# showlab/VideoSwap

Measured on AMD Instinct MI355X. Metric: denoised frames/sec, 16-frame 512x512 clip @ 50 DDIM steps (end to end: inversion + CFG sampling), higher is better.
Workload: dtype f16; 1 GPU; BASELINE.json configs[1]: 16-frame 512x512 clip, SD-1.5 UNet3D + AnimateDiff motion modules, 50-step DDIM inversion (B=1) + 50-step CFG-7.5 DDIM sampling (B=2), 1 clip per GPU per step; launch=eager, parallelism=clip-parallel x1

## Files before the change

include/vsx.h:

```cpp
#ifndef VSX_H_
#define VSX_H_

#include <stddef.h>
#include <stdint.h>

#ifdef __cplusplus
extern "C" {
#endif

#define VSX_ABI_VERSION 13

#define VSX_OK 0
#define VSX_E_BADSHAPE (-1)
#define VSX_E_UNSUPPORTED (-2)
#define VSX_E_LAUNCH (-3)
#define VSX_E_WORKSPACE (-4)

typedef void* vsx_stream_t;

int vsx_abi_version(void);
const char* vsx_last_error(void);
const char* vsx_source_digest(void);
int vsx_set_option(const char* name, int64_t value);

typedef struct vsx_gemm_desc {
    int64_t M, N, K;
    int64_t batch0, batch1;

    const void* A;
    const void* A2;
    int64_t lda, a_bs0, a_bs1;
    int64_t a_mode;
    int64_t H, W;
    int64_t C1, C2;
    int64_t ks, stride;
    int64_t upsample;

    const void* B;
    int64_t ldb, b_bs0, b_bs1;

    void* C;
    int64_t ldc, c_bs0, c_bs1;
    int64_t c_mode;
    int64_t c_rows_per_img;
    int64_t c_img_stride;

    const void* bias;
    const void* rowvec;
    int64_t rows_per_vec;
    const void* residual;
    int64_t ldr, r_bs0, r_bs1;
    int64_t geglu;
    double alpha;
    void* workspace;
    int64_t workspace_bytes;
    int64_t pad_lo, pad_hi;
    const void* rowscale;
    const void* colvec;
    void* rowstats;
    int64_t rowstats_parts;
} vsx_gemm_desc;

int vsx_gemm_f16(const vsx_gemm_desc* d, vsx_stream_t stream);
int64_t vsx_gemm_rowstats_parts(const vsx_gemm_desc* d);
int64_t vsx_gemm_workspace(const vsx_gemm_desc* d);

int64_t vsx_groupnorm_chunks(int64_t rows, int64_t nimg);
int vsx_groupnorm_stats(const void* x1, const void* x2, int64_t nimg, int64_t rows, int64_t C1,
                        int64_t C2, int64_t groups, float* partial, vsx_stream_t stream);
int vsx_groupnorm_apply(const void* x1, const void* x2, int64_t nimg, int64_t rows, int64_t C1,
                        int64_t C2, int64_t groups, const float* partial, int64_t nchunks,
                        int64_t count_rows, const void* gamma, const void* beta, float eps,
                        int64_t silu, float* stats, void* y, vsx_stream_t stream);

int vsx_row_stats(const void* x, int64_t M, int64_t C, float eps, float* stats, vsx_stream_t stream);
int vsx_row_stats_combine(const float* parts, int64_t M, int64_t nparts, int64_t C, float eps, float* stats,
                          vsx_stream_t stream);

int vsx_layernorm(const void* x, int64_t M, int64_t C, const void* gamma, const void* beta,
                  float eps, const void* pe, int64_t rows_per_frame, int64_t frames,
                  int64_t frame_offset, void* y, vsx_stream_t stream);

int vsx_attention_f16(const void* Q, const void* K, const void* VT, void* O, int64_t nb,
                      int64_t heads, int64_t nq, int64_t nk, int64_t d, int64_t ldq, int64_t ldk,
                      int64_t ldvt, int64_t ldo, int64_t q_bs, int64_t k_bs, int64_t vt_bs,
                      int64_t o_bs, int64_t kv_div, float scale, vsx_stream_t stream);

int vsx_attention_lse_f16(const void* Q, const void* K, const void* VT, void* O, float* lse, int64_t lse_ld, int64_t nb,
                          int64_t heads, int64_t nq, int64_t nk, int64_t d, int64_t ldq, int64_t ldk, int64_t ldvt,
                          int64_t ldo, int64_t q_bs, int64_t k_bs, int64_t vt_bs, int64_t o_bs, int64_t kv_div,
                          float scale, vsx_stream_t stream);
int64_t vsx_attention_bwd_supported(int64_t d);
int vsx_attention_bwd_f16(const void* Q, const void* K, const void* V, const void* O, const void* dO, const void* QT,
                          const void* KT, const void* dOT, const float* lse, float* delta, void* dQ, void* dK, void* dV,
                          int64_t nb, int64_t heads, int64_t nq, int64_t nk, int64_t d, int64_t ldtq, int64_t ldtk,
                          int64_t lds, int64_t kv_div, float scale, vsx_stream_t stream);

int vsx_softmax_rows(void* S, int64_t nrows, int64_t ncols, int64_t ld, vsx_stream_t stream);
int vsx_softmax_rows_causal(void* S, int64_t nrows, int64_t ncols, int64_t ld, int64_t rows_per_seq,
                            vsx_stream_t stream);

int vsx_temporal_attention_f16(const void* Q, const void* K, const void* V, void* O, int64_t B,
                               int64_t fq, int64_t fk, int64_t hw, int64_t heads, int64_t d,
                               int64_t ldq, int64_t ldkv, int64_t ldo, float scale,
                               vsx_stream_t stream);

int vsx_silu(const void* x, void* y, int64_t n, vsx_stream_t stream);
int vsx_quick_gelu(const void* x, void* y, int64_t n, vsx_stream_t stream);
int vsx_axpy(const void* a, const void* b, float s, void* y, int64_t n, vsx_stream_t stream);
int vsx_pack_latents(const void* x, void* y, int64_t B, int64_t Cin, int64_t F, int64_t HW,
                     int64_t Cpad, vsx_stream_t stream);
int vsx_unpack_latents(const void* x, void* y, int64_t B, int64_t Cout, int64_t F, int64_t HW,
                       int64_t Cs, vsx_stream_t stream);
int vsx_cfg_ddim_step(const void* x, const void* eps_u, const void* eps_c, float guidance,
                      float alpha_t, float alpha_next, void* out, int64_t n, vsx_stream_t stream);
int vsx_masked_blend(const void* x, const void* src, const void* mask, void* out, int64_t C,
                     int64_t n_sp, vsx_stream_t stream);

int vsx_adapter_scatter(const float* tracks, const int32_t* selected, const void* feat, void* out,
                        int64_t F, int64_t P, int64_t C, int64_t h, int64_t w, float rate,
                        float out_scale, vsx_stream_t stream);

int vsx_prof_enable(int64_t on, int64_t max_samples);
int vsx_prof_pause(int64_t paused);
int vsx_prof_collect(int64_t* n_launches, double* total_ms, double* total_flop);
int vsx_prof_collect_roofline(double peak_flops, double peak_bytes_per_s, int64_t* n_launches, double* total_ms,
                              double* total_flop, double* total_bytes, double* floor_ms, double* byte_bound_ms);

#define VSX_COMM_OP_SEND 1
#define VSX_COMM_OP_RECV 2
#define VSX_COMM_OP_ALLGATHER 3
#define VSX_COMM_OP_ALLREDUCE 4
#define VSX_COMM_OP_LOCAL_COPY 5
#define VSX_COMM_OP_GROUP_START 6
#define VSX_COMM_OP_GROUP_END 7
int vsx_comm_unique_id(void* id128);
int vsx_comm_init(int64_t rank, int64_t nranks, const void* id128);
int vsx_comm_init_recording(int64_t rank, int64_t nranks);
int64_t vsx_comm_recorded(int64_t* out, int64_t capacity);
int64_t vsx_comm_size(void);
int64_t vsx_comm_rank(void);
int vsx_comm_destroy(void);
int vsx_allgather_kv(const void* kv_local, void* kv_all, int64_t batch, int64_t elems_per_batch,
                     vsx_stream_t stream);
int vsx_allgather_f32(const float* local, float* all, int64_t count, vsx_stream_t stream);
int vsx_allreduce_gnstats(float* partial, int64_t count, vsx_stream_t stream);
int vsx_alltoall_f16(const void* send, void* recv, int64_t nouter, int64_t ninner, int64_t block_elems,
                     const int64_t* send_strides, const int64_t* recv_strides, vsx_stream_t stream);

int vsx_geglu_fwd(const void* y2, void* out, int64_t M, int64_t N, vsx_stream_t stream);
int vsx_geglu_bwd(const void* dout, const void* y2, void* dy2, int64_t M, int64_t N, vsx_stream_t stream);
int vsx_silu_bwd(const void* dy, const void* x, void* dx, int64_t n, vsx_stream_t stream);
int64_t vsx_groupnorm_bwd_workspace(int64_t nimg, int64_t rows, int64_t groups);
int vsx_groupnorm_bwd(const void* dy, const void* x1, const void* x2, int64_t nimg, int64_t rows, int64_t C1,
                      int64_t C2, int64_t groups, const void* gamma, const void* beta, float eps, int64_t silu,
                      void* ws, void* dx1, void* dx2, vsx_stream_t stream);
// ... 37 lines not shown
```

videoswap_amd/_lib.py:

```python
import ctypes
import os
from ctypes import POINTER, Structure, c_char_p, c_double, c_float, c_int, c_int32, c_int64, c_void_p

_HERE = os.path.dirname(os.path.abspath(__file__))
VARIANT = os.environ.get('VSX_LIB_VARIANT') or None
LIB_PATH = os.path.join(_HERE, 'lib', 'libvsx.so' if not VARIANT else f'libvsx_{VARIANT}.so')

VSX_ABI_VERSION = 13
VSX_E_UNSUPPORTED = -2


class VsxError(RuntimeError):
    pass


class GemmDesc(Structure):

    def __init__(self, *args, **kwargs):
        super().__init__(*args, **kwargs)
        if 'pad_lo' not in kwargs:
            self.pad_lo = -1
        if 'pad_hi' not in kwargs:
            self.pad_hi = -1

    _fields_ = [
        ('M', c_int64), ('N', c_int64), ('K', c_int64),
        ('batch0', c_int64), ('batch1', c_int64),
        ('A', c_void_p), ('A2', c_void_p),
        ('lda', c_int64), ('a_bs0', c_int64), ('a_bs1', c_int64),
        ('a_mode', c_int64), ('H', c_int64), ('W', c_int64), ('C1', c_int64), ('C2', c_int64),
        ('ks', c_int64), ('stride', c_int64), ('upsample', c_int64),
        ('B', c_void_p), ('ldb', c_int64), ('b_bs0', c_int64), ('b_bs1', c_int64),
        ('C', c_void_p), ('ldc', c_int64), ('c_bs0', c_int64), ('c_bs1', c_int64),
        ('c_mode', c_int64), ('c_rows_per_img', c_int64), ('c_img_stride', c_int64),
        ('bias', c_void_p), ('rowvec', c_void_p), ('rows_per_vec', c_int64),
        ('residual', c_void_p), ('ldr', c_int64), ('r_bs0', c_int64), ('r_bs1', c_int64),
        ('geglu', c_int64), ('alpha', c_double),
        ('workspace', c_void_p), ('workspace_bytes', c_int64),
        ('pad_lo', c_int64), ('pad_hi', c_int64),
        ('rowscale', c_void_p), ('colvec', c_void_p),
        ('rowstats', c_void_p), ('rowstats_parts', c_int64),
    ]


PROTOTYPES = {
    'vsx_abi_version': (c_int, []),
    'vsx_last_error': (c_char_p, []),
    'vsx_source_digest': (c_char_p, []),
    'vsx_set_option': (c_int, [c_char_p, c_int64]),
    'vsx_gemm_f16': (c_int, [POINTER(GemmDesc), c_void_p]),
    'vsx_gemm_workspace': (c_int64, [POINTER(GemmDesc)]),
    'vsx_gemm_rowstats_parts': (c_int64, [POINTER(GemmDesc)]),
    'vsx_groupnorm_chunks': (c_int64, [c_int64, c_int64]),
    'vsx_groupnorm_stats': (c_int, [c_void_p, c_void_p, c_int64, c_int64, c_int64, c_int64, c_int64, c_void_p,
                                    c_void_p]),
    'vsx_groupnorm_apply': (c_int, [c_void_p, c_void_p, c_int64, c_int64, c_int64, c_int64, c_int64, c_void_p,
                                    c_int64, c_int64, c_void_p, c_void_p, c_float, c_int64, c_void_p, c_void_p, c_void_p]),
    'vsx_row_stats': (c_int, [c_void_p, c_int64, c_int64, c_float, c_void_p, c_void_p]),
    'vsx_row_stats_combine': (c_int, [c_void_p, c_int64, c_int64, c_int64, c_float, c_void_p, c_void_p]),
    'vsx_layernorm': (c_int, [c_void_p, c_int64, c_int64, c_void_p, c_void_p, c_float, c_void_p, c_int64, c_int64,
                              c_int64, c_void_p, c_void_p]),
    'vsx_attention_f16': (c_int, [c_void_p, c_void_p, c_void_p, c_void_p] + [c_int64] * 14 + [c_float, c_void_p]),
    'vsx_attention_lse_f16': (c_int, [c_void_p, c_void_p, c_void_p, c_void_p, c_void_p] + [c_int64] * 15 + [c_float, c_void_p]),
    'vsx_attention_bwd_supported': (c_int64, [c_int64]),
    'vsx_attention_bwd_f16': (c_int, [c_void_p] * 13 + [c_int64] * 9 + [c_float, c_void_p]),
    'vsx_softmax_rows': (c_int, [c_void_p, c_int64, c_int64, c_int64, c_void_p]),
    'vsx_softmax_rows_causal': (c_int, [c_void_p, c_int64, c_int64, c_int64, c_int64, c_void_p]),
    'vsx_temporal_attention_f16': (c_int, [c_void_p, c_void_p, c_void_p, c_void_p] + [c_int64] * 9
                                   + [c_float, c_void_p]),
    'vsx_silu': (c_int, [c_void_p, c_void_p, c_int64, c_void_p]),
    'vsx_quick_gelu': (c_int, [c_void_p, c_void_p, c_int64, c_void_p]),
    'vsx_axpy': (c_int, [c_void_p, c_void_p, c_float, c_void_p, c_int64, c_void_p]),
    'vsx_pack_latents': (c_int, [c_void_p, c_void_p, c_int64, c_int64, c_int64, c_int64, c_int64, c_void_p]),
    'vsx_unpack_latents': (c_int, [c_void_p, c_void_p, c_int64, c_int64, c_int64, c_int64, c_int64, c_void_p]),
    'vsx_cfg_ddim_step': (c_int, [c_void_p, c_void_p, c_void_p, c_float, c_float, c_float, c_void_p, c_int64,
                                  c_void_p]),
    'vsx_masked_blend': (c_int, [c_void_p, c_void_p, c_void_p, c_void_p, c_int64, c_int64, c_void_p]),
    'vsx_adapter_scatter': (c_int, [c_void_p, c_void_p, c_void_p, c_void_p, c_int64, c_int64, c_int64, c_int64,
                                    c_int64, c_float, c_float, c_void_p]),
    'vsx_prof_enable': (c_int, [c_int64, c_int64]),
    'vsx_comm_unique_id': (c_int, [c_void_p]),
    'vsx_comm_init': (c_int, [c_int64, c_int64, c_void_p]),
    'vsx_comm_init_recording': (c_int, [c_int64, c_int64]),
    'vsx_comm_recorded': (c_int64, [POINTER(c_int64), c_int64]),
    'vsx_comm_size': (c_int64, []),
    'vsx_comm_rank': (c_int64, []),
    'vsx_comm_destroy': (c_int, []),
    'vsx_allgather_kv': (c_int, [c_void_p, c_void_p, c_int64, c_int64, c_void_p]),
    'vsx_allgather_f32': (c_int, [c_void_p, c_void_p, c_int64, c_void_p]),
    'vsx_allreduce_gnstats': (c_int, [c_void_p, c_int64, c_void_p]),
    'vsx_prof_pause': (c_int, [c_int64]),
    'vsx_prof_collect': (c_int, [POINTER(c_int64), POINTER(c_double), POINTER(c_double)]),
    'vsx_prof_collect_roofline': (c_int, [c_double, c_double, POINTER(c_int64), POINTER(c_double), POINTER(c_double),
                                          POINTER(c_double), POINTER(c_double), POINTER(c_double)]),
    'vsx_geglu_fwd': (c_int, [c_void_p, c_void_p, c_int64, c_int64, c_void_p]),
    'vsx_geglu_bwd': (c_int, [c_void_p, c_void_p, c_void_p, c_int64, c_int64, c_void_p]),
    'vsx_silu_bwd': (c_int, [c_void_p, c_void_p, c_void_p, c_int64, c_void_p]),
    'vsx_groupnorm_bwd_workspace': (c_int64, [c_int64, c_int64, c_int64]),
    'vsx_groupnorm_bwd': (c_int, [c_void_p, c_void_p, c_void_p, c_int64, c_int64, c_int64, c_int64, c_int64, c_void_p,
                                  c_void_p, c_float, c_int64, c_void_p, c_void_p, c_void_p, c_void_p]),
    'vsx_layernorm_bwd': (c_int, [c_void_p, c_void_p, c_void_p, c_float, c_void_p, c_int64, c_int64, c_void_p]),
    'vsx_softmax_bwd': (c_int, [c_void_p, c_void_p, c_int64, c_int64, c_int64, c_float, c_void_p]),
    'vsx_sum_pool2x2': (c_int, [c_void_p, c_void_p, c_int64, c_int64, c_int64, c_int64, c_void_p]),
    'vsx_adapter_gather': (c_int, [c_void_p, c_void_p, c_void_p, c_void_p, c_int64, c_int64, c_int64, c_int64, c_int64,
                                   c_float, c_float, c_void_p]),
    'vsx_alltoall_f16': (c_int, [c_void_p, c_void_p, c_int64, c_int64, c_int64, POINTER(c_int64), POINTER(c_int64),
                                 c_void_p]),
    'vsx_dift_sample_points': (c_int, [c_void_p] + [c_int64] * 7 + [c_void_p, c_int64, c_void_p, c_int64, c_void_p,
                                                                       c_void_p, c_void_p]),
    'vsx_dift_cosine_map_workspace': (c_int64, [c_int64] * 5),
    'vsx_dift_cosine_map': (c_int, [c_void_p] + [c_int64] * 7 + [c_void_p, c_int64, c_int64, c_void_p, c_int64,
                                                                    c_void_p, c_void_p, c_void_p, c_void_p]),
    'vsx_coord_mlp_f32': (c_int, [c_void_p] + [c_int64] * 10 + [c_void_p, c_int64, c_void_p, c_void_p]),
    'vsx_hash_grid_geometry': (c_int64, [c_int64] * 4 + [c_double] + [c_void_p] * 5),
    'vsx_hash_grid_f32': (c_int, [c_void_p, c_int64, c_int64, c_void_p] + [c_int64] * 5 + [c_double, c_void_p, c_void_p]),
    'vsx_hash_mlp_f32': (c_int, [c_void_p, c_int64, c_int64, c_void_p] + [c_int64] * 5 + [c_double] + [c_int64] * 5
                         + [c_void_p, c_int64, c_void_p, c_void_p]),
}

OPTIONAL_PROTOTYPES = {}

_lib = None


def load():
    global _lib
    if _lib is not None:
        return _lib
    if not os.path.exists(LIB_PATH):
        raise VsxError(
            f'{LIB_PATH} not found: the HIP extension is the only implementation of the denoising path; '
            f'build it with `python -m videoswap_amd.build` (hipcc --offload-arch=gfx950).')
    lib = ctypes.CDLL(LIB_PATH)
    for name, (restype, argtypes) in PROTOTYPES.items():
        fn = getattr(lib, name)
        fn.restype = restype
        fn.argtypes = argtypes
    for name, (restype, argtypes) in OPTIONAL_PROTOTYPES.items():
        fn = getattr(lib, name, None)
        if fn is not None:
# ... 22 lines not shown
```

videoswap_amd/csrc/norm.hip:

```cpp
#include "common.h"
#include "options.h"

namespace {

constexpr int GN_MAX_THREADS = 512;
constexpr int GN_MAX_GROUPS = 64;

__host__ __device__ inline int gn_threads(int C) {
    const int vpr = C >> 3;
    return (GN_MAX_THREADS / vpr) * vpr;
}

__host__ __device__ inline int gn_stat_rows(long rows, long nimg) {
    long r = rows * nimg / 768;
    return (int)(r < 8 ? 8 : (r > 1024 ? 1024 : r));
}
__host__ __device__ inline int gn_apply_rows(long rows, long nimg) {
    long r = rows * nimg / 1024;
    return (int)(r < 4 ? 4 : (r > 512 ? 512 : r));
}

__device__ __forceinline__ int gn_col(const int c, const int C) { return ((c >> 2) & 1) * (C >> 1) + (c >> 3) * 4 + (c & 3); }

__device__ __forceinline__ const half_t* gn_src(const half_t* x1, const half_t* x2, int c, int C1, int C2, long& pitch) {
// ... 110 lines not shown
                                                                  const float* __restrict__ stats,
                                                                  const half_t* __restrict__ gamma, const half_t* __restrict__ beta,
                                                                  int silu, half_t* __restrict__ y, const float* __restrict__ partial,
                                                                  int nchunks, float inv_count, float eps, float* __restrict__ stats_out) {
    const int C = C1 + C2;
    const int cpg = C / groups;
    const int vpr = C >> 3;
    const int rp = (int)blockDim.x / vpr;
    const int tid = threadIdx.x;
    const int rl = tid / vpr;
    const int c0 = (tid - rl * vpr) * 8;
    const long img = blockIdx.y;
    __shared__ float st_sh[FUSED ? 2 * GN_MAX_GROUPS : 2];
    if constexpr (FUSED) {
        const int lane = tid & 63, wave = tid >> 6;
        const int nwaves = (int)blockDim.x >> 6;
        if (wave < nwaves) {
            const float2* pp = reinterpret_cast<const float2*>(partial) + img * nchunks * groups;
            for (int g = wave; g < groups; g += nwaves) {
                float2 v = lane < nchunks ? pp[(long)lane * groups + g] : make_float2(0.f, 0.f);
#pragma unroll
                for (int w = 32; w > 0; w >>= 1) {
                    v.x += __shfl_down(v.x, w, 64);
                    v.y += __shfl_down(v.y, w, 64);
                }
                if (lane == 0) {
                    float mean, rstd;
                    gn_mean_rstd(v.x, v.y, inv_count, eps, mean, rstd);
                    st_sh[2 * g] = mean;
                    st_sh[2 * g + 1] = rstd;
                    if (blockIdx.x == 0) {
                        stats_out[(img * groups + g) * 2] = mean;
                        stats_out[(img * groups + g) * 2 + 1] = rstd;
                    }
                }
            }
        }
        __syncthreads();
    }
    float ca[8], cb[8];
    {
        const h8 gm = as_h8(ld16(gamma + c0)), bt = as_h8(ld16(beta + c0));
        const float* st = FUSED ? st_sh : stats + img * groups * 2;
        int g = c0 / cpg, left = (g + 1) * cpg - c0;
        float mean = st[2 * g], rstd = st[2 * g + 1];
#pragma unroll
        for (int e = 0; e < 8; ++e) {
            if (left == 0) { ++g; left = cpg; mean = st[2 * g]; rstd = st[2 * g + 1]; }
            --left;
            ca[e] = rstd * (float)gm[e];
            cb[e] = (float)bt[e] - mean * ca[e];
        }
    }
    long pitch;
    const half_t* src = gn_src(x1, x2, c0, C1, C2, pitch) + img * rows * pitch;
    half_t* dst = y + img * rows * C + c0;
    const int rpb = gn_apply_rows(rows, gridDim.y);
    const long r0 = (long)blockIdx.x * rpb;
    const long r1 = min(r0 + (long)rpb, rows);
    for (long rb = r0 + rl; rb < r1; rb += 4 * rp) {
        uint4 raw[4];
#pragma unroll
        for (int u = 0; u < 4; ++u) {
            const long r = rb + u * rp;
            raw[u] = r < r1 ? ld16(src + r * pitch) : make_uint4(0, 0, 0, 0);
        }
#pragma unroll
        for (int u = 0; u < 4; ++u) {
            const long r = rb + u * rp;
            if (r >= r1) break;
            const h8 v = as_h8(raw[u]);
            h8 o;
#pragma unroll
            for (int e = 0; e < 8; ++e) {
                float f = __builtin_fmaf((float)v[e], ca[e], cb[e]);
                if (silu) f = silu_f(f);
                o[e] = (half_t)f;
            }
            st16(dst + r * C, as_u4(o));
        }
    }
}

template <int NV, int R>
__global__ __launch_bounds__(256) void layernorm_kernel(const half_t* __restrict__ x, long M, int C,
                                                        const half_t* __restrict__ gamma,
                                                        const half_t* __restrict__ beta, float eps,
                                                        const half_t* __restrict__ pe, long rows_per_frame, int frames,
                                                        int frame_offset, half_t* __restrict__ y) {
    const int lane = threadIdx.x & 63;
    const long m0 = ((long)blockIdx.x * 4 + (threadIdx.x >> 6)) * R;
    if (m0 >= M) return;
    const int vpr = C >> 3;
    uint4 raw[R][NV];
#pragma unroll
    for (int r = 0; r < R; ++r)
#pragma unroll
        for (int k = 0; k < NV; ++k) {
            const int v = lane + 64 * k;
            raw[r][k] = (v < vpr && m0 + r < M) ? ld16(x + (m0 + r) * C + v * 8) : make_uint4(0, 0, 0, 0);
        }
    h8 gm[NV], bt[NV];
#pragma unroll
    for (int k = 0; k < NV; ++k) {
        const int v = lane + 64 * k;
        if (v < vpr) {
            gm[k] = as_h8(ld16(gamma + v * 8));
            bt[k] = as_h8(ld16(beta + v * 8));
        }
    }
#pragma unroll
    for (int r = 0; r < R; ++r) {
        const long m = m0 + r;
        if (m >= M) break;
        float f[NV][8];
        float sum = 0.f;
#pragma unroll
        for (int k = 0; k < NV; ++k) {
            const h8 h = as_h8(raw[r][k]);
#pragma unroll
            for (int e = 0; e < 8; ++e) { f[k][e] = (float)h[e]; sum += f[k][e]; }
        }
        const float mean = wave_sum(sum) / (float)C;
        float sq = 0.f;
#pragma unroll
        for (int k = 0; k < NV; ++k) {
            if (lane + 64 * k < vpr) {
#pragma unroll
                for (int e = 0; e < 8; ++e) { const float d = f[k][e] - mean; sq += d * d; }
            }
        }
        const float rstd = rsqrtf(wave_sum(sq) / (float)C + eps);
        const half_t* perow = nullptr;
        if (pe) {
            const long fr = (m / rows_per_frame) % frames + frame_offset;
            perow = pe + fr * C;
        }
#pragma unroll
        for (int k = 0; k < NV; ++k) {
            const int v = lane + 64 * k;
            if (v < vpr) {
                h8 o;
                if (perow) {
                    const h8 pv = as_h8(ld16(perow + v * 8));
#pragma unroll
                    for (int e = 0; e < 8; ++e)
                        o[e] = (half_t)((f[k][e] - mean) * rstd * (float)gm[k][e] + (float)bt[k][e] + (float)pv[e]);
                } else {
#pragma unroll
                    for (int e = 0; e < 8; ++e)
                        o[e] = (half_t)((f[k][e] - mean) * rstd * (float)gm[k][e] + (float)bt[k][e]);
                }
                st16(y + m * C + v * 8, as_u4(o));
            }
        }
    }
}

template <int NV, int R>
__global__ __launch_bounds__(256) void row_stats_kernel(const half_t* __restrict__ x, long M, int C, float eps,
                                                        float* __restrict__ stats) {
    const int lane = threadIdx.x & 63;
    const long m0 = ((long)blockIdx.x * 4 + (threadIdx.x >> 6)) * R;
    if (m0 >= M) return;
    const int vpr = C >> 3;
    uint4 raw[R][NV];
// ... 63 lines not shown
    for (int c = lane; c < ncols; c += 64) sum += __expf((float)row[c] - mx);
    sum = wave_sum(sum);
    const float inv = 1.0f / sum;
    for (int c = lane; c < ncols; c += 64) row[c] = (half_t)(__expf((float)row[c] - mx) * inv);
}

__global__ __launch_bounds__(256) void softmax_rows_causal_kernel(half_t* __restrict__ S, long nrows, int ncols,
                                                                  long ld, int rows_per_seq) {
    const int lane = threadIdx.x & 63;
    const long r = (long)blockIdx.x * 4 + (threadIdx.x >> 6);
    if (r >= nrows) return;
    half_t* row = S + r * ld;
    const int live = min(ncols, (int)(r % rows_per_seq) + 1);
    float mx = -INFINITY;
    for (int c = lane; c < live; c += 64) mx = fmaxf(mx, (float)row[c]);
    mx = wave_max(mx);
    float sum = 0.f;
    for (int c = lane; c < live; c += 64) sum += __expf((float)row[c] - mx);
    sum = wave_sum(sum);
    const float inv = 1.0f / sum;
    for (int c = lane; c < ncols; c += 64) row[c] = c < live ? (half_t)(__expf((float)row[c] - mx) * inv) : (half_t)0.f;
}

}

extern "C" int64_t vsx_groupnorm_chunks(int64_t rows, int64_t nimg) {
    const int rpc = gn_stat_rows(rows, nimg);
    return (rows + rpc - 1) / rpc;
}

static int gn_check(const void* x1, const void* x2, int64_t nimg, int64_t rows, int64_t C1, int64_t C2,
                    int64_t groups) {
    VSX_REQUIRE(x1 && nimg > 0 && rows > 0, VSX_E_BADSHAPE, "groupnorm: empty input");
    VSX_REQUIRE(C1 > 0 && C1 % 8 == 0 && C2 >= 0 && C2 % 8 == 0, VSX_E_BADSHAPE,
                "groupnorm: channels must be multiples of 8 (C1=%ld C2=%ld)", (long)C1, (long)C2);
    VSX_REQUIRE((C2 == 0) == (x2 == nullptr), VSX_E_BADSHAPE, "groupnorm: x2/C2 mismatch");
    const int64_t C = C1 + C2;
    VSX_REQUIRE(C <= 4096, VSX_E_UNSUPPORTED, "groupnorm: C=%ld > 4096", (long)C);
    VSX_REQUIRE(groups > 0 && groups <= GN_MAX_GROUPS && C % groups == 0, VSX_E_BADSHAPE,
                "groupnorm: groups=%ld does not divide C=%ld (max %d groups)", (long)groups, (long)C, GN_MAX_GROUPS);
    VSX_REQUIRE(vsx_aligned16(x1) && vsx_aligned16(x2), VSX_E_BADSHAPE, "groupnorm: inputs must be 16-byte aligned");
    VSX_REQUIRE(nimg <= 65535, VSX_E_BADSHAPE, "groupnorm: nimg=%ld > 65535", (long)nimg);
    return VSX_OK;
}

extern "C" int vsx_groupnorm_stats(const void* x1, const void* x2, int64_t nimg, int64_t rows, int64_t C1,
                                   int64_t C2, int64_t groups, float* partial, vsx_stream_t stream) {
    int rc = gn_check(x1, x2, nimg, rows, C1, C2, groups);
    if (rc) return rc;
    VSX_REQUIRE(partial != nullptr, VSX_E_WORKSPACE, "groupnorm_stats: null partial buffer");
    dim3 grid((unsigned)vsx_groupnorm_chunks(rows, nimg), (unsigned)nimg);
    hipLaunchKernelGGL(gn_stats_kernel, grid, dim3((unsigned)gn_threads((int)(C1 + C2))), 0, (hipStream_t)stream, (const half_t*)x1,
                       (const half_t*)x2, (long)rows, (int)C1, (int)C2, (int)groups, partial);
    return vsx_check_launch("vsx_groupnorm_stats");
}

extern "C" int vsx_groupnorm_apply(const void* x1, const void* x2, int64_t nimg, int64_t rows, int64_t C1,
                                   int64_t C2, int64_t groups, const float* partial, int64_t nchunks,
                                   int64_t count_rows, const void* gamma, const void* beta, float eps, int64_t silu,
                                   float* stats, void* y, vsx_stream_t stream) {
    int rc = gn_check(x1, x2, nimg, rows, C1, C2, groups);
    if (rc) return rc;
    VSX_REQUIRE(partial && gamma && beta && y && stats, VSX_E_BADSHAPE, "groupnorm_apply: null argument");
    VSX_REQUIRE(nchunks > 0 && count_rows > 0, VSX_E_BADSHAPE, "groupnorm_apply: nchunks/count_rows");
    VSX_REQUIRE(vsx_aligned16(gamma) && vsx_aligned16(beta) && vsx_aligned16(y), VSX_E_BADSHAPE,
                "groupnorm_apply: gamma/beta/y must be 16-byte aligned");
    const int64_t C = C1 + C2;
    const float inv_count = 1.0f / ((float)count_rows * (float)(C / groups));
    const int rpb = gn_apply_rows(rows, nimg);
    dim3 grid((unsigned)((rows + rpb - 1) / rpb), (unsigned)nimg);
    const unsigned threads = (unsigned)gn_threads((int)C);
    if (nchunks <= GN_FUSE_MAX_CHUNKS && threads >= 64 && vsxg::gemm_option("gn_fuse") != 0) {
        hipLaunchKernelGGL(gn_apply_kernel<true>, grid, dim3(threads), 0, (hipStream_t)stream, (const half_t*)x1, (const half_t*)x2,
                           (long)rows, (int)C1, (int)C2, (int)groups, (const float*)nullptr, (const half_t*)gamma, (const half_t*)beta,
                           (int)silu, (half_t*)y, partial, (int)nchunks, inv_count, eps, stats);
        return vsx_check_launch("vsx_groupnorm_apply");
    }
    hipLaunchKernelGGL(gn_finalize_kernel, dim3((unsigned)groups, (unsigned)nimg), dim3(256), 0, (hipStream_t)stream, partial,
                       (int)nchunks, (int)groups, inv_count, eps, stats);
    hipLaunchKernelGGL(gn_apply_kernel<false>, grid, dim3(threads), 0, (hipStream_t)stream, (const half_t*)x1, (const half_t*)x2,
                       (long)rows, (int)C1, (int)C2, (int)groups, stats, (const half_t*)gamma, (const half_t*)beta,
                       (int)silu, (half_t*)y, (const float*)nullptr, 0, 0.f, 0.f, (float*)nullptr);
    return vsx_check_launch("vsx_groupnorm_apply");
}

extern "C" int vsx_layernorm(const void* x, int64_t M, int64_t C, const void* gamma, const void* beta, float eps,
                             const void* pe, int64_t rows_per_frame, int64_t frames, int64_t frame_offset, void* y,
                             vsx_stream_t stream) {
    VSX_REQUIRE(x && gamma && beta && y, VSX_E_BADSHAPE, "layernorm: null argument");
    if (M == 0) return VSX_OK;
    VSX_REQUIRE(M > 0 && C > 0 && C % 8 == 0 && C <= 2048, VSX_E_BADSHAPE, "layernorm: C=%ld must be a multiple of 8, <= 2048",
                (long)C);
    VSX_REQUIRE(vsx_aligned16(x) && vsx_aligned16(gamma) && vsx_aligned16(beta) && vsx_aligned16(y) && vsx_aligned16(pe),
                VSX_E_BADSHAPE, "layernorm: pointers must be 16-byte aligned");
    if (pe) VSX_REQUIRE(rows_per_frame > 0 && frames > 0 && frame_offset >= 0, VSX_E_BADSHAPE, "layernorm: pe geometry");
    const long rpf = rows_per_frame > 0 ? rows_per_frame : 1;
    const int nfr = (int)(frames > 0 ? frames : 1);
#define VSX_LN_LAUNCH(NV, R)                                                                                            \
    hipLaunchKernelGGL((layernorm_kernel<NV, R>), dim3((unsigned)((M + 4 * (R) - 1) / (4 * (R)))), dim3(256), 0,            \
                       (hipStream_t)stream, (const half_t*)x, (long)M, (int)C, (const half_t*)gamma,                    \
                       (const half_t*)beta, eps, (const half_t*)pe, rpf, nfr, (int)frame_offset, (half_t*)y)
    if (C <= 512) VSX_LN_LAUNCH(1, 4);
    else if (C <= 1024) VSX_LN_LAUNCH(2, 2);
    else VSX_LN_LAUNCH(4, 1);
#undef VSX_LN_LAUNCH
    return vsx_check_launch("vsx_layernorm");
}

extern "C" int vsx_row_stats(const void* x, int64_t M, int64_t C, float eps, float* stats, vsx_stream_t stream) {
    VSX_REQUIRE(x && stats, VSX_E_BADSHAPE, "row_stats: null argument");
    if (M == 0) return VSX_OK;
    VSX_REQUIRE(M > 0 && C > 0 && C % 8 == 0 && C <= 2048, VSX_E_BADSHAPE, "row_stats: C=%ld must be a multiple of 8, <= 2048",
                (long)C);
    VSX_REQUIRE(vsx_aligned16(x), VSX_E_BADSHAPE, "row_stats: x must be 16-byte aligned");
#define VSX_RS_LAUNCH(NV, R)                                                                                            \
    hipLaunchKernelGGL((row_stats_kernel<NV, R>), dim3((unsigned)((M + 4 * (R) - 1) / (4 * (R)))), dim3(256), 0,            \
                       (hipStream_t)stream, (const half_t*)x, (long)M, (int)C, eps, stats)
    if (C <= 512) VSX_RS_LAUNCH(1, 4);
    else if (C <= 1024) VSX_RS_LAUNCH(2, 2);
    else VSX_RS_LAUNCH(4, 1);
#undef VSX_RS_LAUNCH
    return vsx_check_launch("vsx_row_stats");
}

extern "C" int vsx_row_stats_combine(const float* parts, int64_t M, int64_t nparts, int64_t C, float eps, float* stats,
                                     vsx_stream_t stream) {
    VSX_REQUIRE(parts && stats, VSX_E_BADSHAPE, "row_stats_combine: null argument");
    if (M == 0) return VSX_OK;
    VSX_REQUIRE(M > 0 && nparts > 0 && nparts <= 64 && C > 0, VSX_E_BADSHAPE, "row_stats_combine: M=%ld nparts=%ld C=%ld", (long)M,
                (long)nparts, (long)C);
    VSX_REQUIRE((((uintptr_t)parts) & 7) == 0 && (((uintptr_t)stats) & 7) == 0, VSX_E_BADSHAPE, "row_stats_combine: 8-byte alignment");
    hipLaunchKernelGGL(row_stats_combine_kernel, dim3((unsigned)((M + 255) / 256)), dim3(256), 0, (hipStream_t)stream, parts, (long)M,
                       (int)nparts, 1.0f / (float)C, eps, stats);
    return vsx_check_launch("vsx_row_stats_combine");
}

extern "C" int vsx_softmax_rows(void* S, int64_t nrows, int64_t ncols, int64_t ld, vsx_stream_t stream) {
    VSX_REQUIRE(S != nullptr && ncols > 0 && ld >= ncols, VSX_E_BADSHAPE, "softmax_rows: bad arguments");
    if (nrows == 0) return VSX_OK;
    hipLaunchKernelGGL(softmax_rows_kernel, dim3((unsigned)((nrows + 3) / 4)), dim3(256), 0, (hipStream_t)stream,
                       (half_t*)S, (long)nrows, (int)ncols, (long)ld);
    return vsx_check_launch("vsx_softmax_rows");
}

extern "C" int vsx_softmax_rows_causal(void* S, int64_t nrows, int64_t ncols, int64_t ld, int64_t rows_per_seq,
                                       vsx_stream_t stream) {
    VSX_REQUIRE(S != nullptr && ncols > 0 && ld >= ncols && rows_per_seq > 0, VSX_E_BADSHAPE,
                "softmax_rows_causal: bad arguments");
    if (nrows == 0) return VSX_OK;
    hipLaunchKernelGGL(softmax_rows_causal_kernel, dim3((unsigned)((nrows + 3) / 4)), dim3(256), 0, (hipStream_t)stream,
                       (half_t*)S, (long)nrows, (int)ncols, (long)ld, (int)rows_per_seq);
    return vsx_check_launch("vsx_softmax_rows_causal");
}
```

videoswap_amd/csrc/options.cpp:

```cpp
#include "options.h"

#include <stdlib.h>
#include <string.h>

#include "common.h"

namespace vsxg {
namespace {
struct Option { const char* name; const char* env; long value; bool init; };
Option g_options[] = {{"gemm_pp", "VSX_GEMM_PP", 1, false}, {"pp_sched", "VSX_PP_SCHED", 0, false},
                      {"tile_tune", "VSX_TUNE_TILE", 0, false}, {"xcd_walk", "VSX_XCD_WALK", 1, false},
                      {"attn_qb", "VSX_ATTN_QB", 0, false}, {"temporal_out", "VSX_TEMPORAL_OUT", 0, false},
                      {"attn_o16", "VSX_ATTN_O16", 0, false}, {"gn_fuse", "VSX_GN_FUSE", 0, false},
                      {"gemm_ws", "VSX_GEMM_WS", 1, false}, {"ws_waves", "VSX_WS_WAVES", 10, false}};
Option* find_option(const char* name) {
    for (auto& o : g_options)
        if (strcmp(o.name, name) == 0) {
            if (!o.init) {
                const char* e = getenv(o.env);
                if (e) o.value = atol(e);
                o.init = true;
            }
            return &o;
        }
    return nullptr;
}
}
long gemm_option(const char* name) {
    Option* o = find_option(name);
    return o ? o->value : 0;
}
}

extern "C" int vsx_set_option(const char* name, int64_t value) {
    auto* o = name ? vsxg::find_option(name) : nullptr;
    if (!o) return vsx_fail(VSX_E_BADSHAPE, "vsx_set_option: unknown option '%s'", name ? name : "(null)");
    o->value = (long)value;
    return VSX_OK;
}
```

videoswap_amd/ops.py:

```python
import ctypes
import os

import torch

from . import _lib
from ._lib import GemmDesc, check

_F16 = torch.float16


_raw_stream = getattr(torch._C, '_cuda_getCurrentRawStream', None)


def _stream():
    if _raw_stream is not None:
        return ctypes.c_void_p(_raw_stream(torch.cuda.current_device()))
    return ctypes.c_void_p(torch.cuda.current_stream().cuda_stream)


def _p(t):
    return None if t is None else ctypes.c_void_p(t.data_ptr())


def _chk(t, name, dtype=_F16):
# ... 414 lines not shown
    if probs.dtype != _F16 or not probs.is_cuda:
        raise _lib.VsxError('attention_pv: probs must be an fp16 GPU tensor')
    _chk(vt, 'vt')
    C, ldvt = vt.shape[1], vt.shape[2]
    dh = C // heads
    out = torch.empty(nb, nq, C, dtype=_F16, device=probs.device)
    kred = round_up(nk, 8)
    if ldvt < kred:
        raise _lib.VsxError('attention_pv: vt rows are shorter than round_up(nk, 8)')
    groups = [(0, nb, 0)] if kv_div == 1 else [(kb * kv_div, kv_div, kb) for kb in range(vt.shape[0])]
    for (b0, cnt, kb) in groups:
        d = GemmDesc()
        d.M, d.N, d.K = nq, dh, kred
        d.batch0, d.batch1 = cnt, heads
        d.A = probs[b0:].data_ptr(); d.lda = ld; d.a_bs0 = heads * nq * ld; d.a_bs1 = nq * ld
        d.B = vt[kb if kv_div != 1 else b0:].data_ptr(); d.ldb = ldvt
        d.b_bs0 = 0 if kv_div != 1 else C * ldvt; d.b_bs1 = dh * ldvt
        d.C = out[b0:].data_ptr(); d.ldc = C; d.c_bs0 = nq * C; d.c_bs1 = dh
        d.alpha = 1.0
        gemm(d)
    return out


def _rows_view(t, name):
    _chk_view(t, name)
    if t.dim() != 3 or t.stride(2) != 1 or t.stride(1) % 8 or t.stride(0) % 8 or (t.data_ptr() % 16):
        raise _lib.VsxError(f'{name}: need unit inner stride, 16-byte aligned base, strides multiple of 8 (got {t.stride()})')
    return t.stride(1), t.stride(0)


def _chk_view(t, name):
    if not t.is_cuda or t.dtype != _F16:
        raise _lib.VsxError(f'{name}: expected an fp16 GPU tensor')


def attention(q, k, vt, heads, scale, kv_div=1, nk=None):
    _chk(vt, 'vt')
    ldq, q_bs = _rows_view(q, 'q')
    ldk, k_bs = _rows_view(k, 'k')
    nb, nq, C = q.shape
    nk = k.shape[1] if nk is None else nk
    dh = C // heads
    out = torch.empty(nb, nq, C, dtype=_F16, device=q.device)
    if FlopCounter.enabled:
        FlopCounter.attention += 4.0 * nb * heads * nq * nk * dh
    check(_lib.load().vsx_attention_f16(_p(q), _p(k), _p(vt), _p(out), nb, heads, nq, nk, dh, ldq, ldk, vt.shape[2], C,
                                        q_bs, k_bs, C * vt.shape[2], nq * C, kv_div, float(scale),
                                        _stream()), 'vsx_attention_f16')
    return out


def temporal_attention(q, k, v, B, fq, fk, hw, heads, scale):
    for t, n in ((q, 'q'), (k, 'k'), (v, 'v')):
        _chk_view(t, n)
        if t.dim() != 2 or t.stride(1) != 1 or t.stride(0) % 8 or t.data_ptr() % 16:
            raise _lib.VsxError(f'{n}: need a [rows, C] tensor with unit inner stride and aligned rows')
    if k.stride(0) != v.stride(0):
        raise _lib.VsxError('temporal_attention: k and v must share their row stride')
    C = q.shape[-1]
    out = torch.empty(q.shape[0], C, dtype=_F16, device=q.device)
    if FlopCounter.enabled:
        FlopCounter.attention += 4.0 * B * hw * fq * fk * C
    fn = _lib.load().vsx_temporal_attention_f16
    if fq <= 32 or fk > 128:
        check(fn(_p(q), _p(k), _p(v), _p(out), B, fq, fk, hw, heads, C // heads, q.stride(0), k.stride(0), C,
                 float(scale), _stream()), 'vsx_temporal_attention_f16')
        return out
    for b in range(B):
        kb, vb = k[b * fk * hw:(b + 1) * fk * hw], v[b * fk * hw:(b + 1) * fk * hw]
        for f0 in range(0, fq, 32):
            n = min(32, fq - f0)
            r0 = (b * fq + f0) * hw
            check(fn(_p(q[r0:r0 + n * hw]), _p(kb), _p(vb), _p(out[r0:r0 + n * hw]), 1, n, fk, hw, heads, C // heads,
                     q.stride(0), k.stride(0), C, float(scale), _stream()), 'vsx_temporal_attention_f16')
    return out


def group_norm(x, gamma, beta, groups, eps, nimg, silu=False, x2=None, partial_hook=None, count_rows=None):
    _chk(x, 'x'); _chk(x2, 'x2'); _chk(gamma, 'gamma'); _chk(beta, 'beta')
    C1 = x.shape[-1]
    C2 = x2.shape[-1] if x2 is not None else 0
    rows = x.numel() // C1 // nimg
    lib = _lib.load()
    nchunks = lib.vsx_groupnorm_chunks(rows, nimg)
    partial = torch.empty(nimg, nchunks, groups, 2, dtype=torch.float32, device=x.device)
    s = _stream()
    check(lib.vsx_groupnorm_stats(_p(x), _p(x2), nimg, rows, C1, C2, groups, _p(partial), s), 'vsx_groupnorm_stats')
    if partial_hook is not None:
        partial = partial_hook(partial)
        nchunks = partial.shape[1]
    y = torch.empty(*x.shape[:-1], C1 + C2, dtype=_F16, device=x.device)
    stats = torch.empty(nimg, groups, 2, dtype=torch.float32, device=x.device)
    check(lib.vsx_groupnorm_apply(_p(x), _p(x2), nimg, rows, C1, C2, groups, _p(partial), nchunks,
                                  rows if count_rows is None else count_rows, _p(gamma), _p(beta), float(eps),
                                  1 if silu else 0, _p(stats), _p(y), s), 'vsx_groupnorm_apply')
    return y


def layer_norm(x, gamma, beta, eps=1e-5, pe=None, rows_per_frame=0, frames=0, frame_offset=0):
    if isinstance(x, DeferredLN):
        raise _lib.VsxError('layer_norm of a deferred LayerNorm: materialize() it first')
    _chk(x, 'x'); _chk(gamma, 'gamma'); _chk(beta, 'beta'); _chk(pe, 'pe')
    C = x.shape[-1]
    if pe is not None:
        if pe.dim() != 2 or pe.shape[1] != C or frames <= 0 or rows_per_frame <= 0 or frame_offset < 0 \
                or pe.shape[0] < frame_offset + frames:
            raise _lib.VsxError(f'layer_norm: positional-encoding table {tuple(pe.shape)} does not cover frames '
                                f'[{frame_offset}, {frame_offset + frames}) x {C} channels')
    y = torch.empty_like(x)
    check(_lib.load().vsx_layernorm(_p(x), x.numel() // C, C, _p(gamma), _p(beta), float(eps), _p(pe), rows_per_frame,
                                    frames, frame_offset, _p(y), _stream()), 'vsx_layernorm')
    return y


def silu(x):
    _chk(x, 'x')
    y = torch.empty_like(x)
    check(_lib.load().vsx_silu(_p(x), _p(y), x.numel(), _stream()), 'vsx_silu')
    return y


def quick_gelu(x):
    _chk(x, 'x')
    y = torch.empty_like(x)
    check(_lib.load().vsx_quick_gelu(_p(x), _p(y), x.numel(), _stream()), 'vsx_quick_gelu')
    return y


def axpy(a, b, s=1.0):
    _chk(a, 'a'); _chk(b, 'b')
    if a.shape != b.shape:
        raise _lib.VsxError(f'axpy: shape mismatch {tuple(a.shape)} vs {tuple(b.shape)}')
    y = torch.empty_like(a)
    check(_lib.load().vsx_axpy(_p(a), _p(b), float(s), _p(y), a.numel(), _stream()), 'vsx_axpy')
    return y


def pack_latents(x, cpad=8):
    _chk(x, 'x')
    B, C, F, H, W = x.shape
    y = torch.empty(B * F, H, W, cpad, dtype=_F16, device=x.device)
    check(_lib.load().vsx_pack_latents(_p(x), _p(y), B, C, F, H * W, cpad, _stream()), 'vsx_pack_latents')
    return y


def unpack_latents(x, B, cout):
    _chk(x, 'x')
    BF, H, W, Cs = x.shape
    F = BF // B
    y = torch.empty(B, cout, F, H, W, dtype=_F16, device=x.device)
    check(_lib.load().vsx_unpack_latents(_p(x), _p(y), B, cout, F, H * W, Cs, _stream()), 'vsx_unpack_latents')
    return y


def cfg_ddim_step(x, eps_u, eps_c, guidance, alpha_t, alpha_next):
    _chk(x, 'x'); _chk(eps_u, 'eps_u'); _chk(eps_c, 'eps_c')
    out = torch.empty_like(x)
    check(_lib.load().vsx_cfg_ddim_step(_p(x), _p(eps_u), _p(eps_c), float(guidance), float(alpha_t),
                                        float(alpha_next), _p(out), x.numel(), _stream()), 'vsx_cfg_ddim_step')
    return out


def masked_blend(x, src, mask):
    _chk(x, 'x'); _chk(src, 'src'); _chk(mask, 'mask')
    C = x.shape[0]
    n_sp = x.numel() // C
    if mask.numel() != n_sp or src.shape != x.shape:
        raise _lib.VsxError('masked_blend: shape mismatch')
    out = torch.empty_like(x)
# ... 350 lines not shown
```

Before: 4.149 frames/s.

## Add single-pass register-resident GroupNorm kernel for small slabs

Adds a one-launch GroupNorm kernel in which each workgroup loads a channel slab of an image into registers, reduces the group statistics in-block, and then normalizes (with optional SiLU) from registers. It replaces the two-kernel stats+apply path and the partial-buffer allocation whenever the geometry fits the register budget. The aim is to cut the second global read of the activation and one launch per GroupNorm. The cost is heavy register pressure with up to 21 uint4 values per thread, and possibly fewer workgroups when the image count is small.

New measurement: 4.183 frames/s (median of 6 runs). No clear change (+0.8%).

```diff
diff --git a/include/vsx.h b/include/vsx.h
--- a/include/vsx.h
+++ b/include/vsx.h
@@ -8,7 +8,7 @@
 extern "C" {
 #endif
 
-#define VSX_ABI_VERSION 13
+#define VSX_ABI_VERSION 14
 
 #define VSX_OK 0
 #define VSX_E_BADSHAPE (-1)
@@ -72,6 +72,10 @@
                         int64_t C2, int64_t groups, const float* partial, int64_t nchunks,
                         int64_t count_rows, const void* gamma, const void* beta, float eps,
                         int64_t silu, float* stats, void* y, vsx_stream_t stream);
+int64_t vsx_groupnorm_one_fits(int64_t nimg, int64_t rows, int64_t C1, int64_t C2, int64_t groups);
+int vsx_groupnorm_one(const void* x1, const void* x2, int64_t nimg, int64_t rows, int64_t C1, int64_t C2,
+                      int64_t groups, const void* gamma, const void* beta, float eps, int64_t silu,
+                      float* stats, void* y, vsx_stream_t stream);
 
 int vsx_row_stats(const void* x, int64_t M, int64_t C, float eps, float* stats, vsx_stream_t stream);
 int vsx_row_stats_combine(const float* parts, int64_t M, int64_t nparts, int64_t C, float eps, float* stats,
diff --git a/videoswap_amd/_lib.py b/videoswap_amd/_lib.py
--- a/videoswap_amd/_lib.py
+++ b/videoswap_amd/_lib.py
@@ -6,7 +6,7 @@
 VARIANT = os.environ.get('VSX_LIB_VARIANT') or None
 LIB_PATH = os.path.join(_HERE, 'lib', 'libvsx.so' if not VARIANT else f'libvsx_{VARIANT}.so')
 
-VSX_ABI_VERSION = 13
+VSX_ABI_VERSION = 14
 VSX_E_UNSUPPORTED = -2
 
 
@@ -56,6 +56,9 @@
                                     c_void_p]),
     'vsx_groupnorm_apply': (c_int, [c_void_p, c_void_p, c_int64, c_int64, c_int64, c_int64, c_int64, c_void_p,
                                     c_int64, c_int64, c_void_p, c_void_p, c_float, c_int64, c_void_p, c_void_p, c_void_p]),
+    'vsx_groupnorm_one_fits': (c_int64, [c_int64] * 5),
+    'vsx_groupnorm_one': (c_int, [c_void_p, c_void_p, c_int64, c_int64, c_int64, c_int64, c_int64, c_void_p, c_void_p, c_float,
+                                  c_int64, c_void_p, c_void_p, c_void_p]),
     'vsx_row_stats': (c_int, [c_void_p, c_int64, c_int64, c_float, c_void_p, c_void_p]),
     'vsx_row_stats_combine': (c_int, [c_void_p, c_int64, c_int64, c_int64, c_float, c_void_p, c_void_p]),
     'vsx_layernorm': (c_int, [c_void_p, c_int64, c_int64, c_void_p, c_void_p, c_float, c_void_p, c_int64, c_int64,
diff --git a/videoswap_amd/csrc/norm.hip b/videoswap_amd/csrc/norm.hip
--- a/videoswap_amd/csrc/norm.hip
+++ b/videoswap_amd/csrc/norm.hip
@@ -216,6 +216,171 @@
     }
 }
 
+constexpr int GN_ONE_THREADS = 1024;
+constexpr int GN_ONE_VECTORS = 20;
+constexpr int GN_ONE_PASSES = 21;
+constexpr int GN_ONE_MAX_SLAB_GROUPS = 8;
+
+__device__ __forceinline__ void gn_one_keep_f16(uint4& v, float (&s)[8], float (&q)[8]) {
+#if defined(__AMDGCN__)
+    asm volatile("" : "+v"(v.x), "+v"(v.y), "+v"(v.z), "+v"(v.w), "+v"(s[0]), "+v"(s[1]), "+v"(s[2]), "+v"(s[3]), "+v"(s[4]), "+v"(s[5]),
+                      "+v"(s[6]), "+v"(s[7]), "+v"(q[0]), "+v"(q[1]), "+v"(q[2]), "+v"(q[3]), "+v"(q[4]), "+v"(q[5]), "+v"(q[6]), "+v"(q[7]));
+#else
+    (void)v; (void)s; (void)q;
+#endif
+}
+
+__device__ __forceinline__ void gn_one_sched_fence() {
+#if defined(__AMDGCN__)
+    __builtin_amdgcn_sched_barrier(0);
+#endif
+}
+
+struct GnOneGeom {
+    int S, vps, rp, passes, threads;
+};
+inline bool gn_one_geom(long rows, long C, long groups, GnOneGeom& g) {
+    if (rows <= 0 || C <= 0 || groups <= 0 || C % 8 || C % groups) return false;
+    const long cpg = C / groups;
+    long gcd = 8;
+    while (cpg % gcd) gcd >>= 1;
+    const long S = cpg / gcd * 8;
+    if (C % S || groups % (S / cpg)) return false;
+    const long vps = S / 8;
+    if (vps > GN_ONE_THREADS || rows * vps > (long)GN_ONE_THREADS * GN_ONE_VECTORS) return false;
+    const long rp = GN_ONE_THREADS / vps, passes = (rows + rp - 1) / rp;
+    if (passes > GN_ONE_PASSES) return false;
+    g.S = (int)S;
+    g.vps = (int)vps;
+    g.rp = (int)rp;
+    g.passes = (int)passes;
+    g.threads = (int)(((rows < rp ? rows : rp) * vps + 63) / 64 * 64);
+    return true;
+}
+
+template <int NV, bool SILU>
+__global__ __launch_bounds__(GN_ONE_THREADS) void gn_one_kernel(const half_t* __restrict__ x1, const half_t* __restrict__ x2, int rows,
+                                                                int C1, int C2, int groups, int S, const half_t* __restrict__ gamma,
+                                                                const half_t* __restrict__ beta, float inv_count, float eps,
+                                                                half_t* __restrict__ y, float* __restrict__ stats_out) {
+    __shared__ float red[(GN_ONE_THREADS / 64) * GN_ONE_MAX_SLAB_GROUPS * 2];
+    __shared__ float st_sh[GN_ONE_MAX_SLAB_GROUPS * 2];
+    const int C = C1 + C2;
+    const int cpg = C / groups;
+    const int vps = S >> 3, ng = S / cpg, nslab = C / S;
+    const int rp = GN_ONE_THREADS / vps;
+    int wg = blockIdx.x;
+    {
+        const int nwg = gridDim.x, qq = nwg >> 3, rr = nwg & 7;
+        const int xcd = wg & 7, local = wg >> 3;
+        wg = (xcd < rr ? xcd * (qq + 1) : rr * (qq + 1) + (xcd - rr) * qq) + local;
+    }
+    const int slab = wg % nslab;
+    const long img = wg / nslab;
+    const int tid = threadIdx.x;
+    const int rl = tid / vps;
+    const int cs = (tid - rl * vps) * 8;
+    const int c0 = slab * S + cs;
+    const int nk = (rl < rp && rl < rows) ? (rows - rl + rp - 1) / rp : 0;
+    long pitch_l;
+    const half_t* src = gn_src(x1, x2, c0, C1, C2, pitch_l) + img * rows * pitch_l;
+    const int pitch = (int)pitch_l;
+    const int row0 = nk > 0 ? rl : 0;
+
+    uint4 raw[NV];
+#pragma unroll
+    for (int k = 0; k < NV; ++k) raw[k] = ld16(src + (row0 + (k < nk ? k : 0) * rp) * pitch);
+    gn_one_sched_fence();
+    float s[8], q[8];
+#pragma unroll
+    for (int e = 0; e < 8; ++e) { s[e] = 0.f; q[e] = 0.f; }
+#pragma unroll
+    for (int k = 0; k < NV; ++k) {
+        if (k >= nk) raw[k] = make_uint4(0, 0, 0, 0);
+        const h8 v = as_h8(raw[k]);
+#pragma unroll
+        for (int e = 0; e < 8; ++e) {
+            const float f = (float)v[e];
+            s[e] += f;
+            q[e] += f * f;
+        }
+        gn_one_keep_f16(raw[k], s, q);
+    }
+    const h8 gm = as_h8(ld16(gamma + c0)), bt = as_h8(ld16(beta + c0));
+    const int g0 = cs / cpg;
+    {
+        const int lane = tid & 63, wave = tid >> 6;
+#pragma unroll
+        for (int g = 0; g < GN_ONE_MAX_SLAB_GROUPS; ++g) {
+            if (g >= ng) break;
+            float a = 0.f, b = 0.f;
+            int ge = g0, left = (g0 + 1) * cpg - cs;
+#pragma unroll
+            for (int e = 0; e < 8; ++e) {
+                if (left == 0) { ++ge; left = cpg; }
+                --left;
+                a += ge == g ? s[e] : 0.f;
+                b += ge == g ? q[e] : 0.f;
+            }
+#pragma unroll
+            for (int w = 32; w > 0; w >>= 1) {
+                a += __shfl_down(a, w, 64);
+                b += __shfl_down(b, w, 64);
+            }
+            if (lane == 0) {
+                red[(wave * GN_ONE_MAX_SLAB_GROUPS + g) * 2] = a;
+                red[(wave * GN_ONE_MAX_SLAB_GROUPS + g) * 2 + 1] = b;
+            }
+        }
+    }
+    __syncthreads();
+    if (tid < ng) {
+        const int nwaves = (int)blockDim.x >> 6;
+        float a = 0.f, b = 0.f;
+        for (int w = 0; w < nwaves; ++w) {
+            a += red[(w * GN_ONE_MAX_SLAB_GROUPS + tid) * 2];
+            b += red[(w * GN_ONE_MAX_SLAB_GROUPS + tid) * 2 + 1];
+        }
+        float mean, rstd;
+        gn_mean_rstd(a, b, inv_count, eps, mean, rstd);
+        st_sh[2 * tid] = mean;
+        st_sh[2 * tid + 1] = rstd;
+        if (stats_out) {
+            float* out = stats_out + (img * groups + (long)slab * ng + tid) * 2;
+            out[0] = mean;
+            out[1] = rstd;
+        }
+    }
+    __syncthreads();
+    float ca[8], cb[8];
+    {
+        int g = g0, left = (g0 + 1) * cpg - cs;
+        float mean = st_sh[2 * g], rstd = st_sh[2 * g + 1];
+#pragma unroll
+        for (int e = 0; e < 8; ++e) {
+            if (left == 0) { ++g; left = cpg; mean = st_sh[2 * g]; rstd = st_sh[2 * g + 1]; }
+            --left;
+            ca[e] = rstd * (float)gm[e];
+            cb[e] = (float)bt[e] - mean * ca[e];
+        }
+    }
+    half_t* dst = y + img * rows * C + c0;
+#pragma unroll
+    for (int k = 0; k < NV; ++k) {
+        if (k < nk) {
+            const h8 v = as_h8(raw[k]);
+            h8 o;
+#pragma unroll
+            for (int e = 0; e < 8; ++e) {
+                float f = __builtin_fmaf((float)v[e], ca[e], cb[e]);
+                if (SILU) f = silu_f(f);
+                o[e] = (half_t)f;
+            }
+            st16(dst + (rl + k * rp) * C, as_u4(o));
+        }
+    }
+}
+
 template <int NV, int R>
 __global__ __launch_bounds__(256) void layernorm_kernel(const half_t* __restrict__ x, long M, int C,
                                                         const half_t* __restrict__ gamma,
@@ -445,6 +610,55 @@
                        (long)rows, (int)C1, (int)C2, (int)groups, stats, (const half_t*)gamma, (const half_t*)beta,
                        (int)silu, (half_t*)y, (const float*)nullptr, 0, 0.f, 0.f, (float*)nullptr);
     return vsx_check_launch("vsx_groupnorm_apply");
+}
+
+static bool gn_one_auto(int64_t nimg, int64_t C, const GnOneGeom& g) {
+    return !(g.passes > 16 && nimg * (C / g.S) < 64);
+}
+
+extern "C" int64_t vsx_groupnorm_one_fits(int64_t nimg, int64_t rows, int64_t C1, int64_t C2, int64_t groups) {
+    const long mode = vsxg::gemm_option("gn_one");
+    GnOneGeom g;
+    if (mode == 0 || nimg <= 0 || C1 <= 0 || C2 < 0 || C1 % 8 || C2 % 8 || groups > GN_MAX_GROUPS || C1 + C2 > 4096 || nimg > 65535 ||
+        !gn_one_geom(rows, C1 + C2, groups, g))
+        return 0;
+    return mode >= 2 || gn_one_auto(nimg, C1 + C2, g) ? 1 : 0;
+}
+
+extern "C" int vsx_groupnorm_one(const void* x1, const void* x2, int64_t nimg, int64_t rows, int64_t C1, int64_t C2, int64_t groups,
+                                 const void* gamma, const void* beta, float eps, int64_t silu, float* stats, void* y,
+                                 vsx_stream_t stream) {
+    int rc = gn_check(x1, x2, nimg, rows, C1, C2, groups);
+    if (rc) return rc;
+    VSX_REQUIRE(gamma && beta && y, VSX_E_BADSHAPE, "groupnorm_one: null argument");
+    VSX_REQUIRE(vsx_aligned16(gamma) && vsx_aligned16(beta) && vsx_aligned16(y), VSX_E_BADSHAPE,
+                "groupnorm_one: gamma/beta/y must be 16-byte aligned");
+    const int64_t C = C1 + C2;
+    GnOneGeom g;
+    VSX_REQUIRE(gn_one_geom(rows, C, groups, g), VSX_E_UNSUPPORTED,
+                "groupnorm_one: %ld rows x %ld channels in %ld groups do not fit one workgroup per channel slab", (long)rows, (long)C,
+                (long)groups);
+    const float inv_count = 1.0f / ((float)rows * (float)(C / groups));
+    const dim3 grid((unsigned)(nimg * (C / g.S))), block((unsigned)g.threads);
+#define VSX_GN_ONE_LAUNCH_(NV, SILU)                                                                                               \
+    hipLaunchKernelGGL((gn_one_kernel<NV, SILU>), grid, block, 0, (hipStream_t)stream, (const half_t*)x1, (const half_t*)x2,         \
+                       (int)rows, (int)C1, (int)C2, (int)groups, g.S, (const half_t*)gamma, (const half_t*)beta, inv_count, eps,      \
+                       (half_t*)y, stats)
+#define VSX_GN_ONE_LAUNCH(NV)                    \
+    do {                                         \
+        if (silu) VSX_GN_ONE_LAUNCH_(NV, true);  \
+        else VSX_GN_ONE_LAUNCH_(NV, false);      \
+    } while (0)
+    if (g.passes <= 1) VSX_GN_ONE_LAUNCH(1);
+    else if (g.passes <= 2) VSX_GN_ONE_LAUNCH(2);
+    else if (g.passes <= 4) VSX_GN_ONE_LAUNCH(4);
+    else if (g.passes <= 8) VSX_GN_ONE_LAUNCH(8);
+    else if (g.passes <= 12) VSX_GN_ONE_LAUNCH(12);
+    else if (g.passes <= 16) VSX_GN_ONE_LAUNCH(16);
+    else VSX_GN_ONE_LAUNCH(GN_ONE_PASSES);
+#undef VSX_GN_ONE_LAUNCH
+#undef VSX_GN_ONE_LAUNCH_
+    return vsx_check_launch("vsx_groupnorm_one");
 }
 
 extern "C" int vsx_layernorm(const void* x, int64_t M, int64_t C, const void* gamma, const void* beta, float eps,
diff --git a/videoswap_amd/csrc/options.cpp b/videoswap_amd/csrc/options.cpp
--- a/videoswap_amd/csrc/options.cpp
+++ b/videoswap_amd/csrc/options.cpp
@@ -12,6 +12,7 @@
                       {"tile_tune", "VSX_TUNE_TILE", 0, false}, {"xcd_walk", "VSX_XCD_WALK", 1, false},
                       {"attn_qb", "VSX_ATTN_QB", 0, false}, {"temporal_out", "VSX_TEMPORAL_OUT", 0, false},
                       {"attn_o16", "VSX_ATTN_O16", 0, false}, {"gn_fuse", "VSX_GN_FUSE", 0, false},
+                      {"gn_one", "VSX_GN_ONE", 1, false},
                       {"gemm_ws", "VSX_GEMM_WS", 1, false}, {"ws_waves", "VSX_WS_WAVES", 10, false}};
 Option* find_option(const char* name) {
     for (auto& o : g_options)
diff --git a/videoswap_amd/ops.py b/videoswap_amd/ops.py
--- a/videoswap_amd/ops.py
+++ b/videoswap_amd/ops.py
@@ -520,9 +520,14 @@
     C2 = x2.shape[-1] if x2 is not None else 0
     rows = x.numel() // C1 // nimg
     lib = _lib.load()
+    s = _stream()
+    if partial_hook is None and count_rows in (None, rows) and lib.vsx_groupnorm_one_fits(nimg, rows, C1, C2, groups):
+        y = torch.empty(*x.shape[:-1], C1 + C2, dtype=_F16, device=x.device)
+        check(lib.vsx_groupnorm_one(_p(x), _p(x2), nimg, rows, C1, C2, groups, _p(gamma), _p(beta), float(eps),
+                                    1 if silu else 0, None, _p(y), s), 'vsx_groupnorm_one')
+        return y
     nchunks = lib.vsx_groupnorm_chunks(rows, nimg)
     partial = torch.empty(nimg, nchunks, groups, 2, dtype=torch.float32, device=x.device)
-    s = _stream()
     check(lib.vsx_groupnorm_stats(_p(x), _p(x2), nimg, rows, C1, C2, groups, _p(partial), s), 'vsx_groupnorm_stats')
     if partial_hook is not None:
         partial = partial_hook(partial)
```
